# khuzema-h/marl-gym-pybullet-drones

Measured on NVIDIA B200. Metric: drone_substeps_per_sec, higher is better.
Workload: dtype f32

## Files before the change

include/batch_drones.h:

```cpp
#ifndef BATCH_DRONES_H_
#define BATCH_DRONES_H_

#include <stdint.h>

#ifdef __cplusplus
extern "C" {
#endif

#define BD_VERSION 1

enum { BD_TASK_HOVER = 0, BD_TASK_MULTIHOVER = 1, BD_TASK_SPIRAL = 2,
       BD_TASK_MEETUP = 3, BD_TASK_FLOCK = 4, BD_TASK_LEADERFOLLOWER = 5 };
enum { BD_ACT_RPM = 0, BD_ACT_ONE_D_RPM = 1, BD_ACT_PID = 2, BD_ACT_VEL = 3, BD_ACT_ONE_D_PID = 4 };
enum { BD_MODEL_CF2X = 0, BD_MODEL_CF2P = 1, BD_MODEL_RACE = 2 };
enum { BD_F32 = 0, BD_F64 = 1 };
enum { BD_AERO_GND = 1, BD_AERO_DRAG = 2, BD_AERO_DW = 4 };
enum { BD_INTEGRATOR_QUAT = 0, BD_INTEGRATOR_EULER = 1 };
enum { BD_RESET_FIXED = 0, BD_RESET_JITTER_PHILOX = 1, BD_RESET_JITTER_BUFFER = 2 };

enum {
  BD_OK = 0,
  BD_EINVAL = -1,
  BD_ECUDA = -2,
  BD_ENOMEM = -3
// ... 58 lines not shown
int bd_set_step_many_mode(bd_handle* h, int mode);
int bd_stream_gate(const uint32_t* flag_mapped, void* stream);

int bd_get_rng_state(const bd_handle* h, uint64_t* state4);
int bd_set_rng_state(bd_handle* h, const uint64_t* state4);

int bd_debug_set_tile_epoch(bd_handle* h, int tile, int value, void* stream);

int bd_get_state(bd_handle* h, void* state20_dev, void* rates_dev, int32_t* step_counter_dev,
                 void* stream);

int bd_set_state(bd_handle* h, const void* kin13_dev, const void* targets_dev,
                 const int32_t* step_counter_dev, void* stream);

int bd_get_targets(bd_handle* h, void* targets_dev, void* stream);

int bd_episode_stats(bd_handle* h, double* stats3_dev, int reset, void* stream);

int bd_get_controller_state(bd_handle* h, void* ctrl9_dev, void* stream);
int bd_set_controller_state(bd_handle* h, const void* ctrl9_dev, void* stream);

int bd_set_action_f32(bd_handle* h, int is_f32);

int bd_obs_dim(const bd_handle* h);
int bd_act_dim(const bd_handle* h);
int bd_action_buffer_size(const bd_handle* h);
int bd_substeps(const bd_handle* h);
int64_t bd_launch_count(const bd_handle* h);
const char* bd_last_error(void);
int bd_version(void);

typedef struct bd_actor bd_actor;
int bd_actor_create(int obs_dim, int hidden, int act_dim, int device, bd_actor** out);
void bd_actor_destroy(bd_actor* a);
int bd_actor_set_weights(bd_actor* a, const float* w1, const float* b1, const float* w2, const float* b2,
                         const float* w3, const float* b3, const float* logstd, void* stream);
int bd_actor_forward(bd_actor* a, const float* obs_dev, int64_t rows, const float* noise_dev, uint64_t seed,
                     uint64_t offset, float* act_dev, float* logp_dev, float* mean_dev, void* stream);
int bd_actor_set_trace(bd_actor* a, long long* trace_dev);
int bd_actor_set_input_norm(bd_actor* a, const float* mean_dev, const float* rstd_dev, int period, float clip);
int64_t bd_actor_launch_count(const bd_actor* a);
const char* bd_actor_last_error(void);

typedef struct bd_rms bd_rms;
int bd_rms_create(int cols, int device, double count0, double eps, bd_rms** out);
void bd_rms_destroy(bd_rms* r);
// ... 59 lines not shown
```

marl_gym_pybullet_drones_b200/_native.py:

```python
from __future__ import annotations

import ctypes as C
import os

_HERE = os.path.dirname(os.path.abspath(__file__))
LIB_PATH = os.path.join(_HERE, "libbatchdrones.so")

BD_TASK = {"hover": 0, "multihover": 1, "spiral": 2, "meetup": 3, "flock": 4, "leaderfollower": 5}
BD_ACT = {"rpm": 0, "one_d_rpm": 1, "pid": 2, "vel": 3, "one_d_pid": 4}
BD_MODEL = {"cf2x": 0, "cf2p": 1, "racer": 2}
BD_PRECISION = {"fp32": 0, "fp64": 1}
BD_INTEGRATOR = {"quat": 0, "euler": 1}
BD_RESET = {"fixed": 0, "jitter_philox": 1, "jitter_buffer": 2}

EXPORTS = (
    "bd_create", "bd_destroy", "bd_set_init_poses", "bd_set_jitter", "bd_reset", "bd_step",
    "bd_step_host", "bd_step_host_compact", "bd_step_many", "bd_set_step_many_mode", "bd_stream_gate", "bd_get_rng_state", "bd_set_rng_state",
    "bd_debug_set_tile_epoch", "bd_get_state", "bd_set_state", "bd_get_targets", "bd_episode_stats",
    "bd_get_controller_state", "bd_set_controller_state", "bd_set_action_f32", "bd_obs_dim", "bd_act_dim",
    "bd_action_buffer_size", "bd_substeps", "bd_launch_count", "bd_last_error", "bd_version",
    "bd_actor_create", "bd_actor_destroy", "bd_actor_set_weights", "bd_actor_forward", "bd_actor_set_trace", "bd_actor_launch_count",
    "bd_actor_last_error", "bd_actor_set_input_norm",
    "bd_rms_create", "bd_rms_destroy", "bd_rms_update", "bd_rms_batch_moments", "bd_rms_merge_moments", "bd_rms_normalize", "bd_rms_get", "bd_rms_set",
    "bd_rms_launch_count", "bd_rms_last_error",
    "bd_ppo_net_create", "bd_ppo_net_destroy", "bd_ppo_net_param_count", "bd_ppo_net_stats", "bd_ppo_net_pack", "bd_ppo_forward", "bd_ppo_sample", "bd_ppo_set_trace", "bd_ppo_set_train_mode", "bd_ppo_set_forward_mode",
    "bd_ppo_grad", "bd_ppo_adam_step", "bd_ppo_gae", "bd_ppo_adv_stats", "bd_ppo_launch_count", "bd_ppo_last_error",
    "bd_peer_create", "bd_peer_destroy", "bd_peer_handle_size", "bd_peer_get_handle", "bd_peer_open", "bd_peer_data", "bd_peer_allreduce",
    "bd_peer_unmap", "bd_peer_launch_count", "bd_peer_last_error",
)


class BdConfig(C.Structure):

    _fields_ = [
        ("struct_size", C.c_int32), ("device", C.c_int32),
        ("n_envs", C.c_int32), ("n_drones", C.c_int32),
        ("task", C.c_int32), ("act_type", C.c_int32), ("drone_model", C.c_int32),
        ("precision", C.c_int32), ("aero_flags", C.c_int32), ("integrator", C.c_int32),
        ("pyb_freq", C.c_int32), ("ctrl_freq", C.c_int32),
        ("auto_reset", C.c_int32), ("reset_mode", C.c_int32),
        ("action_is_f32", C.c_int32), ("keep_ang_vel", C.c_int32),
# ... 54 lines not shown
    lib.bd_get_rng_state.argtypes = [vp, C.POINTER(C.c_uint64)]
    lib.bd_get_rng_state.restype = C.c_int
    lib.bd_set_rng_state.argtypes = [vp, C.POINTER(C.c_uint64)]
    lib.bd_set_rng_state.restype = C.c_int
    lib.bd_debug_set_tile_epoch.argtypes = [vp, C.c_int, C.c_int, vp]
    lib.bd_debug_set_tile_epoch.restype = C.c_int
    lib.bd_get_state.argtypes = [vp, vp, vp, vp, vp]
    lib.bd_get_state.restype = C.c_int
    lib.bd_set_state.argtypes = [vp, vp, vp, vp, vp]
    lib.bd_set_state.restype = C.c_int
    lib.bd_get_targets.argtypes = [vp, vp, vp]
    lib.bd_get_targets.restype = C.c_int
    lib.bd_episode_stats.argtypes = [vp, vp, C.c_int, vp]
    lib.bd_episode_stats.restype = C.c_int
    lib.bd_get_controller_state.argtypes = [vp, vp, vp]
    lib.bd_get_controller_state.restype = C.c_int
    lib.bd_set_controller_state.argtypes = [vp, vp, vp]
    lib.bd_set_controller_state.restype = C.c_int
    lib.bd_set_action_f32.argtypes = [vp, C.c_int]
    lib.bd_set_action_f32.restype = C.c_int
    for name in ("bd_obs_dim", "bd_act_dim", "bd_action_buffer_size", "bd_substeps"):
        getattr(lib, name).argtypes = [vp]
        getattr(lib, name).restype = C.c_int
    lib.bd_launch_count.argtypes = [vp]
    lib.bd_launch_count.restype = C.c_int64
    lib.bd_last_error.argtypes = []
    lib.bd_last_error.restype = C.c_char_p
    lib.bd_version.argtypes = []
    lib.bd_version.restype = C.c_int
    lib.bd_actor_create.argtypes = [C.c_int, C.c_int, C.c_int, C.c_int, C.POINTER(vp)]
    lib.bd_actor_create.restype = C.c_int
    lib.bd_actor_destroy.argtypes = [vp]
    lib.bd_actor_destroy.restype = None
    lib.bd_actor_set_weights.argtypes = [vp] + [vp] * 7 + [vp]
    lib.bd_actor_set_weights.restype = C.c_int
    lib.bd_actor_forward.argtypes = [vp, vp, C.c_int64, vp, C.c_uint64, C.c_uint64, vp, vp, vp, vp]
    lib.bd_actor_forward.restype = C.c_int
    lib.bd_actor_set_trace.argtypes = [vp, vp]
    lib.bd_actor_set_trace.restype = C.c_int
    lib.bd_actor_launch_count.argtypes = [vp]
    lib.bd_actor_launch_count.restype = C.c_int64
    lib.bd_actor_last_error.argtypes = []
    lib.bd_actor_last_error.restype = C.c_char_p
    lib.bd_actor_set_input_norm.argtypes = [vp, vp, vp, C.c_int, C.c_float]
    lib.bd_actor_set_input_norm.restype = C.c_int
    lib.bd_rms_create.argtypes = [C.c_int, C.c_int, C.c_double, C.c_double, C.POINTER(vp)]
# ... 81 lines not shown
```

marl_gym_pybullet_drones_b200/csrc/bd_api.cu:

```cuda
#include <cuda_runtime.h>
#include <math.h>
#include <stdarg.h>
#include <stdio.h>
#include <stdlib.h>
#include <string.h>

#include <new>
#include <vector>

#include "../../include/batch_drones.h"
#include "bd_params.h"

namespace {

thread_local char g_err[512] = "";

int fail(int code, const char* fmt, ...) {
  va_list ap;
  va_start(ap, fmt);
  vsnprintf(g_err, sizeof(g_err), fmt, ap);
  va_end(ap);
  return code;
}

// ... 15 lines not shown
  }
  ~DeviceGuard() {
    if (prev >= 0 && prev != target) cudaSetDevice(prev);
  }
  int target = -1;
};

}

struct bd_handle {
  bd_config cfg;
  int S = 0, A = 0, B = 0, D = 0, E = 0;
  int EW = 1;
  long long n_total = 0;
  size_t real = 4;
  bd::LaunchSpec spec{};
  void *s0 = nullptr, *s1 = nullptr, *s2 = nullptr, *s3 = nullptr, *s4 = nullptr;
  float* hist = nullptr;
  int* stepc = nullptr;
  int* gsteps = nullptr;
  int* tile_epoch = nullptr;
  unsigned long long* finished = nullptr;
  int pipeline = 0;
  float* ep_ret = nullptr;
  double* ep_acc = nullptr;
  void* ctrl = nullptr;
  void* init_xyz = nullptr;
  void* init_rpy = nullptr;
  int init_env_stride = 0;
  void* jitter = nullptr;
  void* h_actions = nullptr;
  float* h_obs = nullptr;
  void* h_reward = nullptr;
  uint8_t *h_term = nullptr, *h_trunc = nullptr;
  float* h_tobs = nullptr;
  cudaStream_t hs_a = nullptr, hs_b = nullptr;
  cudaEvent_t hs_start = nullptr, hs_done = nullptr, hs_chunk[8] = {};
  int64_t launches = 0;
  long long total_steps = 0;
  bool graph_mode = false;
  int reset_epoch = 0;
  uint32_t philox_base = 0;
  int many_mode = 0;
  bool poisoned = false;
  int* c_blockcnt = nullptr;
  int* c_total = nullptr;
// ... 1 lines not shown
  float* c_rows_dev = nullptr;
  int c_cap_dev = 0;
  cudaEvent_t hs_compact = nullptr;
  int* c_host[2] = {nullptr, nullptr};
  float* c_rows_host[2] = {nullptr, nullptr};
  int c_cap[2] = {0, 0};
  int c_flip = 0;
  bd::Params<float> pf{};
  bd::Params<double> pd{};
};

namespace {

template <typename R>
void fill_params(const bd_handle* h, bd::Params<R>& P) {
  const bd_config& c = h->cfg;
  using R4 = typename bd::V4<R>::type;
  P.N = c.n_envs; P.M = c.n_drones; P.S = h->S; P.A = h->A; P.B = h->B; P.D = h->D;
  P.E = h->E; P.EW = h->EW; P.n_total = h->n_total;
  P.s0 = (R4*)h->s0; P.s1 = (R4*)h->s1; P.s2 = (R4*)h->s2; P.s3 = (R4*)h->s3; P.s4 = (R4*)h->s4;
  P.hist = h->hist; P.stepc = h->stepc; P.gsteps = h->gsteps; P.tile_epoch = h->tile_epoch; P.finished = h->finished;
  P.step_tiles = h->spec.impl == 1 ? (h->cfg.n_envs + 4 * h->EW - 1) / (4 * h->EW) : (h->cfg.n_envs + h->E - 1) / h->E;
  P.pipeline = h->pipeline; P.pipe_wait = 0; P.early_prefetch = 0; P.ep_ret = h->ep_ret; P.ep_acc = h->ep_acc;
  P.ctrl = (R*)h->ctrl;
  P.act_type = c.act_type; P.ctrl_reset = c.ctrl_reset_on_reset;
  P.ctrl_dt = (R)(1.0 / c.ctrl_freq);
  P.ctrl_gravity = (R)(c.g * c.ctrl_mass);
  P.ctrl_4kf = (R)(4 * c.ctrl_kf);
  P.speed_limit = (R)c.speed_limit; P.speed_limit_f = (float)c.speed_limit;
  P.init_xyz = (const R*)h->init_xyz; P.init_rpy = (const R*)h->init_rpy;
  P.init_env_stride = h->init_env_stride;
  P.jitter = (const R*)h->jitter;
  P.actions = nullptr; P.obs = nullptr; P.reward = nullptr; P.terminated = nullptr;
  P.truncated = nullptr; P.terminal_obs = nullptr; P.reset_mask = nullptr;
  const double gravity = c.g * c.mass;
  const double hover_rpm = sqrt(gravity / (4 * c.kf));
  const double max_rpm = sqrt((c.thrust2weight * gravity) / (4 * c.kf));
  const double max_thrust = 4 * c.kf * max_rpm * max_rpm;
  const double gnd_h_clip =
      0.25 * c.prop_radius * sqrt((15 * max_rpm * max_rpm * c.kf * c.gnd_eff_coeff) / max_thrust);
  P.dt = (R)(1.0 / c.pyb_freq);
  P.hover_rpm = (R)hover_rpm;
  P.kf = (R)c.kf; P.km = (R)c.km;
  P.arm = (R)(c.drone_model == BD_MODEL_CF2P ? c.arm : c.arm / sqrt(2.0));
  P.inv_m = (R)(1.0 / c.mass);
  P.gravity = (R)gravity;
// ... 183 lines not shown
  h->spec.device = cfg->device;
  const bool swarm = cfg->task >= BD_TASK_MEETUP;
  h->spec.generic = (cfg->aero_flags != 0 || cfg->integrator != BD_INTEGRATOR_QUAT || cfg->keep_ang_vel || pid_act || swarm) ? 1 : 0;
  {
    const int m = cfg->n_drones;
    const bool pow2 = (m & (m - 1)) == 0 && m <= 32;
    h->EW = m <= 32 ? 32 / m : 1;
    const char* force = getenv("BD_STEP_IMPL");
    const bool plain = cfg->integrator == BD_INTEGRATOR_QUAT && !cfg->keep_ang_vel;
    h->spec.impl = (cfg->precision == BD_F32 && plain && m <= 32 && (pow2 || !swarm) && !pid_act) ? 1 : 0;
    if (force && strcmp(force, "cta") == 0) h->spec.impl = 0;
    const char* pdl = getenv("BD_PDL");
    h->spec.pdl = (pdl && strcmp(pdl, "0") == 0) ? 0 : 1;
    const char* pl = getenv("BD_PIPELINE");
    h->pipeline = (h->spec.pdl && !(pl && strcmp(pl, "0") == 0)) ? 1 : 0;
  }

  const size_t smem = bd::step_smem_bytes(cfg->precision, h->A, h->B, h->D, cfg->task);
  cudaDeviceProp prop;
  cudaError_t pe = cudaGetDeviceProperties(&prop, cfg->device);
  if (pe != cudaSuccess) { delete h; return fail(BD_ECUDA, "cudaGetDeviceProperties: %s", cudaGetErrorString(pe)); }
  if (h->spec.impl == 1 && (size_t)(4 * h->EW) * cfg->n_drones * h->D * 4 > prop.sharedMemPerBlockOptin) h->spec.impl = 0;
  h->spec.sm_count = prop.multiProcessorCount;
  if (smem > prop.sharedMemPerBlockOptin) {
    delete h;
    return fail(BD_EINVAL, "bd_create: the history staging tile needs %zu B of shared memory (> %zu)", smem,
                (size_t)prop.sharedMemPerBlockOptin);
  }

  const size_t plane = (size_t)h->n_total * 4 * h->real;
  cudaError_t e = cudaSuccess;
  auto alloc = [&](void** p, size_t bytes) {
    if (e == cudaSuccess) e = cudaMalloc(p, bytes);
    if (e == cudaSuccess) e = cudaMemset(*p, 0, bytes);
  };
  alloc(&h->s0, plane); alloc(&h->s1, plane); alloc(&h->s2, plane); alloc(&h->s3, plane);
  if (cfg->keep_ang_vel) alloc(&h->s4, plane);
  alloc((void**)&h->hist, (size_t)h->B * h->n_total * h->A * sizeof(float));
  alloc((void**)&h->stepc, (size_t)cfg->n_envs * sizeof(int));
  alloc((void**)&h->gsteps, 16 * sizeof(int));
  alloc((void**)&h->tile_epoch, (size_t)epoch_tiles(h) * sizeof(int));
  alloc((void**)&h->finished, sizeof(unsigned long long));
  if (cfg->track_episodes) alloc((void**)&h->ep_ret, (size_t)cfg->n_envs * sizeof(float));
  alloc((void**)&h->ep_acc, 3 * sizeof(double));
  if (pid_act) alloc(&h->ctrl, (size_t)bd::kCtrlPlanesHost * h->n_total * h->real);
  if (e != cudaSuccess) {
// ... 476 lines not shown
  if (!h) return fail(BD_EINVAL, "bd_set_action_f32: null handle");
  if (h->cfg.precision == BD_F32 && !is_f32)
    return fail(BD_EINVAL, "bd_set_action_f32: BD_F32 handles take float actions only");
  h->cfg.action_is_f32 = is_f32 ? 1 : 0;
  if (h->h_actions) {
    DeviceGuard guard(h->cfg.device);
    cudaFree(h->h_actions); cudaFree(h->h_obs); cudaFree(h->h_reward); cudaFree(h->h_term); cudaFree(h->h_trunc);
    h->h_actions = nullptr; h->h_obs = nullptr; h->h_reward = nullptr; h->h_term = nullptr; h->h_trunc = nullptr;
  }
  refresh_params(h);
  return BD_OK;
}

int bd_episode_stats(bd_handle* h, double* stats3_dev, int reset, void* stream) {
  if (!h) return fail(BD_EINVAL, "bd_episode_stats: null handle");
  if (!h->ep_ret) return fail(BD_EINVAL, "bd_episode_stats: the handle was created with track_episodes = 0");
  DeviceGuard guard(h->cfg.device);
  cudaError_t e = bd::launch_episode_stats(h->ep_acc, stats3_dev, reset, (cudaStream_t)stream);
  h->launches++;
  if (e != cudaSuccess) return fail(BD_ECUDA, "episode_stats kernel launch failed: %s", cudaGetErrorString(e));
  return BD_OK;
}

int bd_obs_dim(const bd_handle* h) { return h ? h->D : BD_EINVAL; }
int bd_act_dim(const bd_handle* h) { return h ? h->A : BD_EINVAL; }
int bd_action_buffer_size(const bd_handle* h) { return h ? h->B : BD_EINVAL; }
int bd_substeps(const bd_handle* h) { return h ? h->S : BD_EINVAL; }
int64_t bd_launch_count(const bd_handle* h) { return h ? h->launches : 0; }

}
```

marl_gym_pybullet_drones_b200/csrc/bd_device.cuh:

```cuda
#pragma once
#include <cuda_runtime.h>
#include <math.h>
#include <stdint.h>

#include "bd_params.h"

namespace bd {

enum { TASK_HOVER = 0, TASK_MULTIHOVER = 1, TASK_SPIRAL = 2,
       TASK_SWARM = 3, TASK_MEETUP = 3, TASK_FLOCK = 4, TASK_LEADERFOLLOWER = 5 };
enum { MODEL_CF2X = 0, MODEL_CF2P = 1, MODEL_RACE = 2 };
enum { AERO_GND = 1, AERO_DRAG = 2, AERO_DW = 4 };
enum { RESET_FIXED = 0, RESET_PHILOX = 1, RESET_BUFFER = 2 };

__device__ __forceinline__ float  sqrt_(float x)  { return sqrtf(x); }
__device__ __forceinline__ double sqrt_(double x) { return sqrt(x); }
__device__ __forceinline__ float  exp_(float x)  { return expf(x); }
__device__ __forceinline__ double exp_(double x) { return exp(x); }
__device__ __forceinline__ float  atan2_(float y, float x)  { return atan2f(y, x); }
__device__ __forceinline__ double atan2_(double y, double x) { return atan2(y, x); }
__device__ __forceinline__ float  asin_(float x)  { return asinf(x); }
__device__ __forceinline__ double asin_(double x) { return asin(x); }
__device__ __forceinline__ void sincos_(float x, float* s, float* c)  { sincosf(x, s, c); }
__device__ __forceinline__ void sincos_(double x, double* s, double* c) { sincos(x, s, c); }
__device__ __forceinline__ float  abs_(float x)  { return fabsf(x); }
__device__ __forceinline__ double abs_(double x) { return fabs(x); }

__device__ __forceinline__ float4  make4(float a, float b, float c, float d)   { return make_float4(a, b, c, d); }
__device__ __forceinline__ double4 make4(double a, double b, double c, double d) { return make_double4(a, b, c, d); }

template <int BYTES>
__device__ __forceinline__ void cp_async(void* smem_dst, const void* gmem_src) {
  unsigned d = static_cast<unsigned>(__cvta_generic_to_shared(smem_dst));
  if constexpr (BYTES == 16) {
    asm volatile("cp.async.cg.shared.global [%0], [%1], 16;\n" ::"r"(d), "l"(gmem_src) : "memory");
  } else {
    asm volatile("cp.async.ca.shared.global [%0], [%1], %2;\n" ::"r"(d), "l"(gmem_src), "n"(BYTES) : "memory");
  }
}
__device__ __forceinline__ void cp_async_commit() { asm volatile("cp.async.commit_group;\n" ::: "memory"); }
__device__ __forceinline__ void cp_async_wait_all() { asm volatile("cp.async.wait_group 0;\n" ::: "memory"); }

__device__ __forceinline__ void philox4x32_10(uint32_t c[4], uint32_t k0, uint32_t k1) {
#pragma unroll
  for (int r = 0; r < 10; ++r) {
    const uint32_t hi0 = __umulhi(0xD2511F53u, c[0]), lo0 = 0xD2511F53u * c[0];
    const uint32_t hi1 = __umulhi(0xCD9E8D57u, c[2]), lo1 = 0xCD9E8D57u * c[2];
    const uint32_t n0 = hi1 ^ c[1] ^ k0, n2 = hi0 ^ c[3] ^ k1;
    c[0] = n0; c[1] = lo1; c[2] = n2; c[3] = lo0;
    k0 += 0x9E3779B9u; k1 += 0xBB67AE85u;
  }
}
__device__ __forceinline__ float  u01(uint32_t a, uint32_t, float)  { return (a >> 8) * (1.0f / 16777216.0f); }
__device__ __forceinline__ double u01(uint32_t a, uint32_t b, double) {
  return ((a >> 5) * 67108864.0 + (b >> 6)) * (1.0 / 9007199254740992.0);
}

template <typename R>
__device__ __forceinline__ void quat_to_mat(R x, R y, R z, R w, R m[9]) {
  const R d = x * x + y * y + z * z + w * w;
// ... 618 lines not shown
    R ir = clip_(c[3 + k] - re[k] * dt, R(-1500), R(1500));
    if (k < 2) ir = clip_(ir, R(-1), R(1));
    c[3 + k] = ir;
    const R itor = k == 2 ? R(500) : R(0);
    tq[k] = clip_((-(ptor[k] * re[k]) + dtor[k] * rate_e) + itor * ir, R(-3200), R(3200));
  }
  const R mix[4][3] = {{R(-.5), R(-.5), R(-1)}, {R(-.5), R(.5), R(1)}, {R(.5), R(.5), R(-1)}, {R(.5), R(-.5), R(1)}};
#pragma unroll
  for (int k = 0; k < 4; ++k) {
    const R pwm = clip_(thrust + ((mix[k][0] * tq[0] + mix[k][1] * tq[1]) + mix[k][2] * tq[2]), R(20000), R(65535));
    rpm[k] = R(0.2685) * pwm + R(4070.3);
  }
}

__device__ __forceinline__ void bulk_store_s2g(void* gdst, const void* ssrc, uint32_t bytes) {
  const unsigned s = static_cast<unsigned>(__cvta_generic_to_shared(ssrc));
  uint64_t policy;
  asm volatile("createpolicy.fractional.L2::evict_first.b64 %0, 1.0;\n" : "=l"(policy));
  asm volatile("cp.async.bulk.global.shared::cta.bulk_group.L2::cache_hint [%0], [%1], %2, %3;\n" ::"l"(gdst), "r"(s),
               "r"(bytes), "l"(policy)
               : "memory");
  asm volatile("cp.async.bulk.commit_group;\n" ::: "memory");
}
__device__ __forceinline__ void bulk_wait_read0() { asm volatile("cp.async.bulk.wait_group.read 0;\n" ::: "memory"); }
__device__ __forceinline__ void bulk_wait_all0() { asm volatile("cp.async.bulk.wait_group 0;\n" ::: "memory"); }
__device__ __forceinline__ void fence_proxy_async_smem() { asm volatile("fence.proxy.async.shared::cta;\n" ::: "memory"); }

template <int A, bool VEC>
__device__ __forceinline__ void history_run(float*& dst, const float* src, size_t plane, int n) {
#pragma unroll 2
  for (int j = 0; j < n; ++j) {
    if constexpr (VEC) cp_async<16>(dst, src);
    else {
#pragma unroll
      for (int k = 0; k < A; ++k) cp_async<4>(dst + k, src + k);
    }
    dst += A;
    src += plane;
  }
}

template <typename R, int A, bool VEC>
__device__ __forceinline__ void issue_history(const Params<R>& P, long long g, int head, float* myrow,
                                              int j0, int j1) {
  if (g < P.n_total) {
    const size_t plane = (size_t)P.n_total * A;
    const float* base = P.hist + (size_t)g * A;
    float* dst = myrow + 12 + j0 * A;
    const int s0 = head + 1 + j0;
    const int n = j1 - j0;
    if (s0 >= P.B) {
      history_run<A, VEC>(dst, base + (size_t)(s0 - P.B) * plane, plane, n);
    } else {
      const int n1 = min(n, P.B - s0);
      history_run<A, VEC>(dst, base + (size_t)s0 * plane, plane, n1);
      history_run<A, VEC>(dst, base, plane, n - n1);
    }
  }
}

__device__ __forceinline__ int ld_acquire_gpu(const int* p) {
  int v;
  asm volatile("ld.acquire.gpu.global.s32 %0, [%1];\n" : "=r"(v) : "l"(p) : "memory");
  return v;
}
__device__ __forceinline__ int ld_relaxed_gpu(const int* p) {
  int v;
  asm volatile("ld.relaxed.gpu.global.s32 %0, [%1];\n" : "=r"(v) : "l"(p) : "memory");
  return v;
}
__device__ __forceinline__ unsigned long long ld_relaxed_gpu_u64(const unsigned long long* p) {
  unsigned long long v;
  asm volatile("ld.relaxed.gpu.global.u64 %0, [%1];\n" : "=l"(v) : "l"(p) : "memory");
  return v;
}
__device__ __forceinline__ void st_release_gpu(int* p, int v) {
  asm volatile("st.release.gpu.global.s32 [%0], %1;\n" ::"l"(p), "r"(v) : "memory");
}

// ... 38 lines not shown
```

marl_gym_pybullet_drones_b200/csrc/bd_params.h:

```cpp
#pragma once
#include <cuda_runtime.h>
#include <stdint.h>

namespace bd {

constexpr int kBlock = 128;
constexpr int kMaxDrones = 128;
constexpr int kMaxJitterTries = 64;
constexpr int kCtrlPlanesHost = 13;

template <typename Real> struct V4;
template <> struct V4<float>  { using type = float4;  };
template <> struct V4<double> { using type = double4; };

template <typename Real>
struct Params {
  int N, M, S, A, B, D, E;
  int EW;
  long long n_total;
  typename V4<Real>::type *s0, *s1, *s2, *s3, *s4;
  float* hist;
  int* stepc;
  int* gsteps;
  float* ep_ret;
// ... 17 lines not shown
  Real sp_R, sp_omega, sp_vz, sp_cx, sp_cy;
  double pyb_freq, episode_len;
  int trunc_counter;
  int model, aero, integrator, auto_reset, reset_mode, action_is_f32, keep_angv;
  int task;
  int act_type, ctrl_reset;
  Real ctrl_dt, ctrl_gravity, ctrl_4kf, speed_limit;
  float speed_limit_f;
  int host_total;
  int host_head;
  int total_wrap;
  int* tile_epoch;
  unsigned long long* finished;
  long long step_tiles;
  int pipeline;
  int pipe_wait;
  int early_prefetch;
  int block0, grid_blocks;
  int advance;
  int reset_epoch;
  unsigned long long seed;
  int obs_aligned;
  uint32_t philox_base;
};

struct LaunchSpec {
  int task, act_a, precision, generic, device;
  int pdl;
  int impl;
  int sm_count;
};

cudaError_t launch_step_tile(int task, int act_a, const Params<float>& P, const LaunchSpec& ls, cudaStream_t st);
cudaError_t launch_step_tile_many(int task, int act_a, const Params<float>& P, int k, long long act_step, long long obs_step,
                                  long long out_step, const LaunchSpec& ls, cudaStream_t st);
cudaError_t launch_step(const LaunchSpec& ls, const void* params, cudaStream_t st);
cudaError_t launch_reset(const LaunchSpec& ls, const void* params, cudaStream_t st);
cudaError_t launch_get_state(int precision, const void* params, void* state20, void* rates,
                             int32_t* step_counter, cudaStream_t st);
cudaError_t launch_set_state(int precision, const void* params, const void* kin13,
                             const void* targets, const int32_t* step_counter, cudaStream_t st);
cudaError_t launch_get_targets(int precision, const void* params, void* targets, cudaStream_t st);
cudaError_t launch_ctrl_state(int precision, const void* params, void* dst, const void* src, int write,
                              cudaStream_t st);
cudaError_t launch_episode_stats(double* ep_acc, double* out3, int reset, cudaStream_t st);
size_t step_smem_bytes(int precision, int A, int B, int D, int task);
// ... 8 lines not shown
```

marl_gym_pybullet_drones_b200/csrc/bd_step_tile.cuh:

```cuda
#pragma once
#include "bd_device.cuh"

namespace bd {

template <int A>
struct TileIn {
  float4 s0, s1, s2, s3;
  float4 act;
  int stepc;
  float ep_ret;
};

template <int A>
__device__ __forceinline__ void load_state(const Params<float>& P, long long g, int env, bool active, TileIn<A>& in) {
  if (active) {
    in.s0 = P.s0[g]; in.s1 = P.s1[g]; in.s2 = P.s2[g]; in.s3 = P.s3[g];
    in.stepc = P.stepc[env];
    in.ep_ret = P.ep_ret != nullptr ? P.ep_ret[env] : 0.f;
  } else {
    in.s0 = in.s1 = in.s2 = in.s3 = make_float4(0.f, 0.f, 0.f, 0.f);
    in.s1.z = 1.0f;
    in.stepc = 0;
    in.ep_ret = 0.f;
  }
}
template <int A>
__device__ __forceinline__ void load_action(const Params<float>& P, long long g, bool active, TileIn<A>& in) {
  if (active) {
    if constexpr (A == 4) in.act = reinterpret_cast<const float4*>(P.actions)[g];
    else in.act = make_float4(reinterpret_cast<const float*>(P.actions)[g], 0.f, 0.f, 0.f);
  } else {
    in.act = make_float4(0.f, 0.f, 0.f, 0.f);
  }
}

__device__ __forceinline__ float swarm_reward_shfl(const Params<float>& P, const Drone<float>& d, float roll, float pitch,
                                                   int lane, int M, int drone, int& flags) {
  const unsigned full = 0xffffffffu;
  const int base = lane & ~(M - 1);
  const bool tilt = fabsf(roll) > .4f || fabsf(pitch) > .4f;
  flags = 0;
  float contrib = 0.f;
  if (P.task == TASK_MEETUP) {
    const int src = base | (M - 1 - drone);
    const float ox = __shfl_sync(full, d.px, src), oy = __shfl_sync(full, d.py, src), oz = __shfl_sync(full, d.pz, src);
    if (drone < M / 2) {
      const float dx = d.px - ox, dy = d.py - oy, dz = d.pz - oz;
      const float dist = sqrtf(dx * dx + dy * dy + dz * dz);
      contrib = (-1.f * (dist * dist)) * 2.f;
      if (dist > 0.1f) flags |= 4;
    }
    if (fabsf(d.px) > 5.0f || fabsf(d.py) > 5.0f || d.pz > 3.0f || d.pz < 0.1f || tilt) flags |= 2;
  } else if (P.task == TASK_LEADERFOLLOWER) {
// ... 53 lines not shown
}

template <int TASK, int A, bool VEC, int AERO>
__global__ void __launch_bounds__(kBlock, 6)
step_kernel_tile(const __grid_constant__ Params<float> P) {
  extern __shared__ __align__(128) unsigned char smem_raw[];
  const int tid = threadIdx.x, lane = tid & 31;
  const int M = P.M, B = P.B, D = P.D, EW = P.EW;
  const bool pow2 = (M & (M - 1)) == 0;
  constexpr bool vec = VEC;
  float* tile_s = reinterpret_cast<float*>(smem_raw);
  const int env_w = pow2 ? (lane >> (31 - __clz(M))) : lane / M;
  const int group_base = env_w * M;
  const int drone = lane - group_base;
  const int tile = blockIdx.x + P.block0;
  const int env_l = (tid >> 5) * EW + env_w;
  const int env = tile * (4 * EW) + env_l;
  const bool active = env_w < EW && env < P.N;
  const long long g0 = (long long)tile * (4 * EW) * M;
  const long long g = (long long)env * M + drone;
  float* myrow = tile_s + (size_t)(env_w < EW ? env_l * M + drone : 0) * D;
  const bool jit = (TASK == TASK_MULTIHOVER) && (P.reset_mode != RESET_FIXED);
  const long long gh = active ? g : P.n_total;

  pdl_launch_dependents();
  int total, head;
  const bool pipe = P.pipe_wait && P.host_total >= 0;
  if (pipe) {
    total = P.host_total;
    head = P.host_head;
    if (pipe_gate(P, tile, total, tid)) pdl_wait();
    issue_history<float, A, VEC>(P, gh, head, myrow, 0, B - 2);
  } else if (P.host_total >= 0 && P.early_prefetch) {
    total = P.host_total;
    head = P.host_head;
    issue_history<float, A, VEC>(P, gh, head, myrow, 0, B - 2);
    pdl_wait();
  } else {
    pdl_wait();
    total = P.host_total >= 0 ? P.host_total : P.gsteps[0];
    head = total % B;
    issue_history<float, A, VEC>(P, gh, head, myrow, 0, B - 2);
  }
  TileIn<A> cur;
  load_state<A>(P, g, env, active, cur);
  issue_history<float, A, VEC>(P, gh, head, myrow, B - 2, B - 1);
  cp_async_commit();
  load_action<A>(P, g, active, cur);
  const int stepc = cur.stepc;
  float last_sum = 0.f;
  if constexpr (AERO == 2) {
    if ((P.aero & AERO_DRAG) && active && stepc > 0) {
      const int prev = head == 0 ? B - 1 : head - 1;
      const float* lp = P.hist + ((size_t)prev * P.n_total + g) * A;
      if constexpr (A == 4) {
        const float4 pa = *reinterpret_cast<const float4*>(lp);
        last_sum = (__fadd_rn(1.0f, __fmul_rn(0.05f, pa.x)) + __fadd_rn(1.0f, __fmul_rn(0.05f, pa.y))) +
                   (__fadd_rn(1.0f, __fmul_rn(0.05f, pa.z)) + __fadd_rn(1.0f, __fmul_rn(0.05f, pa.w)));
      } else {
        last_sum = 4.0f * __fadd_rn(1.0f, __fmul_rn(0.05f, lp[0]));
      }
    }
  }

  Drone<float> d;
  d.px = cur.s0.x; d.py = cur.s0.y; d.pz = cur.s0.z; d.qx = cur.s0.w;
  d.qy = cur.s1.x; d.qz = cur.s1.y; d.qw = cur.s1.z; d.vx = cur.s1.w;
  d.vy = cur.s2.x; d.vz = cur.s2.y; d.wx = cur.s2.z; d.wy = cur.s2.w;
  d.wz = cur.s3.x; d.tx = cur.s3.y; d.ty = cur.s3.z; d.tz = cur.s3.w;
  float onep[4];
  if constexpr (A == 4) {
// ... 8 lines not shown
  float avx = 0.f, avy = 0.f, avz = 0.f;
  fast_substeps<AERO>(P, d, onep, avx, avy, avz, group_base, drone, last_sum);
  float roll, pitch, yaw;
  quat_to_euler_fast(d.qx, d.qy, d.qz, d.qw, roll, pitch, yaw);

  cp_async_wait_all();
  float contrib = 0.f;
  int flags = 0;
  if (active) {
    if (vec) {
      float4* r4 = reinterpret_cast<float4*>(myrow);
      r4[0] = make_float4(d.px, d.py, d.pz, roll);
      r4[1] = make_float4(pitch, yaw, d.vx, d.vy);
      r4[2] = make_float4(d.vz, avx, avy, avz);
    } else {
      myrow[0] = d.px; myrow[1] = d.py; myrow[2] = d.pz; myrow[3] = roll; myrow[4] = pitch; myrow[5] = yaw;
      myrow[6] = d.vx; myrow[7] = d.vy; myrow[8] = d.vz; myrow[9] = avx; myrow[10] = avy; myrow[11] = avz;
    }
    if constexpr (TASK != TASK_SWARM)
      task_terms<float, TASK>(P, d, roll, pitch, stepc, drone, myrow + 12 + B * A, contrib, flags);
    if constexpr (A == 4) {
      if (vec) *reinterpret_cast<float4*>(myrow + 12 + (B - 1) * 4) = cur.act;
      else { float* o = myrow + 12 + (B - 1) * 4; o[0] = cur.act.x; o[1] = cur.act.y; o[2] = cur.act.z; o[3] = cur.act.w; }
      *reinterpret_cast<float4*>(P.hist + ((size_t)head * P.n_total + g) * 4) = cur.act;
    } else {
      myrow[12 + B - 1] = cur.act.x;
      P.hist[(size_t)head * P.n_total + g] = cur.act.x;
    }
  }

  float swarm_reward_env = 0.f;
  if constexpr (TASK == TASK_SWARM) {
    int fl = 0;
    swarm_reward_env = swarm_reward_shfl(P, d, roll, pitch, lane, M, drone, fl);
    flags = active ? fl : 0;
  }
  if (pow2) {
#pragma unroll 1
    for (int o = M >> 1; o > 0; o >>= 1) {
      contrib += __shfl_xor_sync(0xffffffffu, contrib, o);
      flags |= __shfl_xor_sync(0xffffffffu, flags, o);
    }
  } else {
    const float c0 = contrib;
    const int f0 = flags;
#pragma unroll 1
    for (int o = 1; o < M; ++o) {
      int t = drone + o;
      t -= (t >= M) ? M : 0;
      contrib += __shfl_sync(0xffffffffu, c0, group_base + t);
      flags |= __shfl_sync(0xffffffffu, f0, group_base + t);
    }
  }
  const float reward = (TASK == TASK_SWARM) ? swarm_reward_env : ((TASK == TASK_HOVER) ? contrib : contrib / (float)M);
  const bool time_up = stepc >= P.trunc_counter;
  const bool terminated = (TASK == TASK_SWARM) ? (P.task == TASK_MEETUP && (flags & 4) == 0) : (flags & 1) != 0;
  const bool truncated = ((flags & 2) != 0) || time_up;
  const bool done_reset = active && (terminated || truncated) && P.auto_reset;
  if (active && drone == 0) {
    P.reward[env] = reward;
    P.terminated[env] = terminated ? 1 : 0;
    P.truncated[env] = truncated ? 1 : 0;
    P.stepc[env] = done_reset ? 0 : stepc + P.S;
    if (P.ep_ret != nullptr) {
      float ep = cur.ep_ret + reward;
      if (terminated || truncated) {
        atomicAdd(P.ep_acc + 0, (double)ep);
        atomicAdd(P.ep_acc + 1, (double)(stepc / P.S + 1));
        atomicAdd(P.ep_acc + 2, 1.0);
        ep = 0.f;
      }
      P.ep_ret[env] = ep;
    }
  }

  if (__any_sync(0xffffffffu, done_reset)) {
    float cx = 0.f, cy = 0.f, cz = 0.f;
    if (jit) {
      const long long ib = (long long)env * P.init_env_stride + drone * 3;
      bool retry = done_reset;
#pragma unroll 1
      for (int attempt = 0; attempt <= kMaxJitterTries; ++attempt) {
        const bool last = attempt == kMaxJitterTries;
        if (retry) {
          float j0 = 0.f, j1 = 0.f, j2 = 0.f;
          if (!last) {
            if (P.reset_mode == RESET_BUFFER && P.jitter != nullptr) {
              j0 = P.jitter[g * 3]; j1 = P.jitter[g * 3 + 1]; j2 = P.jitter[g * 3 + 2];
            } else {
              uint32_t c[4] = {(uint32_t)env, (uint32_t)total + P.philox_base, (uint32_t)(attempt * M + drone), 0u};
              uint32_t c2[4] = {c[0], c[1], c[2], 1u};
              philox4x32_10(c, (uint32_t)P.seed, (uint32_t)(P.seed >> 32));
              philox4x32_10(c2, (uint32_t)P.seed, (uint32_t)(P.seed >> 32));
              j0 = -0.25f + 0.5f * u01(c[0], c[1], 0.f);
              j1 = -0.25f + 0.5f * u01(c[2], c[3], 0.f);
// ... 42 lines not shown
      for (int k = 0; k < 12; ++k) myrow[k] = kin[k];
      if (TASK == TASK_SPIRAL) {
        float rp[3], rv[3], sphi, cphi;
        spiral_reference(P, 0, drone, rp, rv, sphi, cphi);
        spiral_extras(myrow + 12 + B * A, d, rp, rv, sphi, cphi);
      }
    }
  }

  const long long left = P.n_total - g0;
  const int tile_rows = 4 * EW * M;
  const int rows = (int)(left < (long long)tile_rows ? left : (long long)tile_rows);
  const uint32_t bytes = (uint32_t)rows * (uint32_t)D * 4u;
  float* gobs = P.obs + (size_t)g0 * D;
  const bool bulk = P.obs_aligned && (bytes & 15u) == 0;
  if (bulk) fence_proxy_async_smem();
  __syncthreads();
  if (bulk) {
    if (tid == 0) bulk_store_s2g(gobs, tile_s, bytes);
  } else {
    for (int i = tid; i < rows * D; i += kBlock) gobs[i] = tile_s[i];
  }
  if (active) {
    P.s0[g] = make_float4(d.px, d.py, d.pz, d.qx);
    P.s1[g] = make_float4(d.qy, d.qz, d.qw, d.vx);
    P.s2[g] = make_float4(d.vy, d.vz, d.wx, d.wy);
    P.s3[g] = make_float4(d.wz, d.tx, d.ty, d.tz);
  }
  if (P.pipeline) {
    __syncthreads();
    if (tid == 0) {
      if (bulk) bulk_wait_all0();
      if (P.host_total >= 0) {
        if (tile == 0) P.gsteps[0] = (total + 1 >= P.total_wrap) ? 0 : total + 1;
      } else {
        const unsigned ticket = atomicAdd(reinterpret_cast<unsigned*>(P.gsteps + 1), 1u);
        if (ticket == gridDim.x - 1) {
          P.gsteps[1] = 0;
          if (P.advance) P.gsteps[0] = (total + 1 >= P.total_wrap) ? 0 : total + 1;
        }
      }
      st_release_gpu(P.tile_epoch + tile, total + 1);
      atomicAdd(P.finished, 1ull);
    }
    return;
  }
  if (tid == 0) {
    const unsigned ticket = atomicAdd(reinterpret_cast<unsigned*>(P.gsteps + 1), 1u);
    if (ticket == gridDim.x - 1) {
      P.gsteps[1] = 0;
// ... 287 lines not shown
```

Measured before the change: 61.04 billion.

## Add L2 cache eviction-priority hints for state, action history and actions

Adds a host-side planner that sizes how much persistent drone state and how many action-history slots fit in about 30% of L2, and per-access createpolicy cache hints in the step-tile kernel. State loads and stores and recent history slots get evict_last, older slots and the one-time action reads get evict_first, so data reused on the next step stays resident in L2 instead of being refetched from HBM. The hinted loads use inline PTX with volatile asm and memory clobbers, which may limit compiler scheduling. The policy can be overridden through the BD_L2_KEEP environment variable.

Measured after the change: 64.81 billion, median of 6. +6.2%, better.

```diff
diff --git a/include/batch_drones.h b/include/batch_drones.h
--- a/include/batch_drones.h
+++ b/include/batch_drones.h
@@ -104,6 +104,10 @@
 
 int bd_set_action_f32(bd_handle* h, int is_f32);
 
+int bd_l2_plan(int n_envs, int n_drones, int act_dim, int buf_slots, int track_episodes, int64_t l2_bytes,
+               const char* force, int* keep_state, int* keep_slots);
+int bd_l2_policy(const bd_handle* h, int* keep_state, int* keep_slots);
+
 int bd_obs_dim(const bd_handle* h);
 int bd_act_dim(const bd_handle* h);
 int bd_action_buffer_size(const bd_handle* h);
diff --git a/marl_gym_pybullet_drones_b200/_native.py b/marl_gym_pybullet_drones_b200/_native.py
--- a/marl_gym_pybullet_drones_b200/_native.py
+++ b/marl_gym_pybullet_drones_b200/_native.py
@@ -16,7 +16,7 @@
 EXPORTS = (
     "bd_create", "bd_destroy", "bd_set_init_poses", "bd_set_jitter", "bd_reset", "bd_step",
     "bd_step_host", "bd_step_host_compact", "bd_step_many", "bd_set_step_many_mode", "bd_stream_gate", "bd_get_rng_state", "bd_set_rng_state",
-    "bd_debug_set_tile_epoch", "bd_get_state", "bd_set_state", "bd_get_targets", "bd_episode_stats",
+    "bd_debug_set_tile_epoch", "bd_l2_plan", "bd_l2_policy", "bd_get_state", "bd_set_state", "bd_get_targets", "bd_episode_stats",
     "bd_get_controller_state", "bd_set_controller_state", "bd_set_action_f32", "bd_obs_dim", "bd_act_dim",
     "bd_action_buffer_size", "bd_substeps", "bd_launch_count", "bd_last_error", "bd_version",
     "bd_actor_create", "bd_actor_destroy", "bd_actor_set_weights", "bd_actor_forward", "bd_actor_set_trace", "bd_actor_launch_count",
@@ -117,6 +117,11 @@
     for name in ("bd_obs_dim", "bd_act_dim", "bd_action_buffer_size", "bd_substeps"):
         getattr(lib, name).argtypes = [vp]
         getattr(lib, name).restype = C.c_int
+    ip = C.POINTER(C.c_int)
+    lib.bd_l2_plan.argtypes = [C.c_int, C.c_int, C.c_int, C.c_int, C.c_int, C.c_int64, C.c_char_p, ip, ip]
+    lib.bd_l2_plan.restype = C.c_int
+    lib.bd_l2_policy.argtypes = [vp, ip, ip]
+    lib.bd_l2_policy.restype = C.c_int
     lib.bd_launch_count.argtypes = [vp]
     lib.bd_launch_count.restype = C.c_int64
     lib.bd_last_error.argtypes = []
diff --git a/marl_gym_pybullet_drones_b200/csrc/bd_api.cu b/marl_gym_pybullet_drones_b200/csrc/bd_api.cu
--- a/marl_gym_pybullet_drones_b200/csrc/bd_api.cu
+++ b/marl_gym_pybullet_drones_b200/csrc/bd_api.cu
@@ -61,6 +61,7 @@
   int* tile_epoch = nullptr;
   unsigned long long* finished = nullptr;
   int pipeline = 0;
+  int l2_keep_state = 0, l2_keep_slots = 0;
   float* ep_ret = nullptr;
   double* ep_acc = nullptr;
   void* ctrl = nullptr;
@@ -108,6 +109,7 @@
   P.hist = h->hist; P.stepc = h->stepc; P.gsteps = h->gsteps; P.tile_epoch = h->tile_epoch; P.finished = h->finished;
   P.step_tiles = h->spec.impl == 1 ? (h->cfg.n_envs + 4 * h->EW - 1) / (4 * h->EW) : (h->cfg.n_envs + h->E - 1) / h->E;
   P.pipeline = h->pipeline; P.pipe_wait = 0; P.early_prefetch = 0; P.ep_ret = h->ep_ret; P.ep_acc = h->ep_acc;
+  P.l2_keep_state = h->l2_keep_state; P.l2_keep_slots = h->l2_keep_slots;
   P.ctrl = (R*)h->ctrl;
   P.act_type = c.act_type; P.ctrl_reset = c.ctrl_reset_on_reset;
   P.ctrl_dt = (R)(1.0 / c.ctrl_freq);
@@ -337,6 +339,11 @@
   if (pe != cudaSuccess) { delete h; return fail(BD_ECUDA, "cudaGetDeviceProperties: %s", cudaGetErrorString(pe)); }
   if (h->spec.impl == 1 && (size_t)(4 * h->EW) * cfg->n_drones * h->D * 4 > prop.sharedMemPerBlockOptin) h->spec.impl = 0;
   h->spec.sm_count = prop.multiProcessorCount;
+  if (h->spec.impl == 1) {
+    const int rc = bd_l2_plan(cfg->n_envs, cfg->n_drones, h->A, h->B, cfg->track_episodes, prop.l2CacheSize,
+                              getenv("BD_L2_KEEP"), &h->l2_keep_state, &h->l2_keep_slots);
+    if (rc) { delete h; return rc; }
+  }
   if (smem > prop.sharedMemPerBlockOptin) {
     delete h;
     return fail(BD_EINVAL, "bd_create: the history staging tile needs %zu B of shared memory (> %zu)", smem,
@@ -859,6 +866,44 @@
   return BD_OK;
 }
 
+int bd_l2_plan(int n_envs, int n_drones, int act_dim, int buf_slots, int track_episodes, int64_t l2_bytes,
+               const char* force, int* keep_state, int* keep_slots) {
+  if (!keep_state || !keep_slots) return fail(BD_EINVAL, "bd_l2_plan: null output");
+  if (n_envs < 1 || n_drones < 1 || act_dim < 1 || buf_slots < 1 || l2_bytes < 0)
+    return fail(BD_EINVAL, "bd_l2_plan: bad shape");
+  *keep_state = 0;
+  *keep_slots = 0;
+  if (force && *force) {
+    if (strcmp(force, "off") == 0) return BD_OK;
+    *keep_state = 1;
+    if (strcmp(force, "state") == 0) return BD_OK;
+    char* end = nullptr;
+    const long k = strtol(force, &end, 10);
+    if (end == force || *end != '\0' || k < 0) {
+      *keep_state = 0;
+      return fail(BD_EINVAL, "BD_L2_KEEP=%s: expected off, state or a slot count", force);
+    }
+    *keep_slots = (int)(k < buf_slots - 1 ? k : buf_slots - 1);
+    return BD_OK;
+  }
+  const long long n = (long long)n_envs * n_drones;
+  const long long state = n * 64 + (long long)n_envs * (track_episodes ? 8 : 4);
+  const long long slot = n * act_dim * 4;
+  const long long budget = l2_bytes * 3 / 10;
+  if (state > budget) return BD_OK;
+  *keep_state = 1;
+  const long long k = (budget - state) / slot;
+  *keep_slots = (int)(k < buf_slots - 1 ? k : buf_slots - 1);
+  return BD_OK;
+}
+
+int bd_l2_policy(const bd_handle* h, int* keep_state, int* keep_slots) {
+  if (!h || !keep_state || !keep_slots) return fail(BD_EINVAL, "bd_l2_policy: null argument");
+  *keep_state = h->l2_keep_state;
+  *keep_slots = h->l2_keep_slots;
+  return BD_OK;
+}
+
 int bd_obs_dim(const bd_handle* h) { return h ? h->D : BD_EINVAL; }
 int bd_act_dim(const bd_handle* h) { return h ? h->A : BD_EINVAL; }
 int bd_action_buffer_size(const bd_handle* h) { return h ? h->B : BD_EINVAL; }
diff --git a/marl_gym_pybullet_drones_b200/csrc/bd_device.cuh b/marl_gym_pybullet_drones_b200/csrc/bd_device.cuh
--- a/marl_gym_pybullet_drones_b200/csrc/bd_device.cuh
+++ b/marl_gym_pybullet_drones_b200/csrc/bd_device.cuh
@@ -36,6 +36,16 @@
     asm volatile("cp.async.cg.shared.global [%0], [%1], 16;\n" ::"r"(d), "l"(gmem_src) : "memory");
   } else {
     asm volatile("cp.async.ca.shared.global [%0], [%1], %2;\n" ::"r"(d), "l"(gmem_src), "n"(BYTES) : "memory");
+  }
+}
+template <int BYTES>
+__device__ __forceinline__ void cp_async_hint(void* smem_dst, const void* gmem_src, uint64_t pol) {
+  unsigned d = static_cast<unsigned>(__cvta_generic_to_shared(smem_dst));
+  if constexpr (BYTES == 16) {
+    asm volatile("cp.async.cg.shared.global.L2::cache_hint [%0], [%1], 16, %2;\n" ::"r"(d), "l"(gmem_src), "l"(pol) : "memory");
+  } else {
+    asm volatile("cp.async.ca.shared.global.L2::cache_hint [%0], [%1], %2, %3;\n" ::"r"(d), "l"(gmem_src), "n"(BYTES), "l"(pol)
+                 : "memory");
   }
 }
 __device__ __forceinline__ void cp_async_commit() { asm volatile("cp.async.commit_group;\n" ::: "memory"); }
@@ -700,39 +710,108 @@
                : "memory");
   asm volatile("cp.async.bulk.commit_group;\n" ::: "memory");
 }
+__device__ __forceinline__ uint64_t l2_pol_last() {
+  uint64_t p;
+  asm("createpolicy.fractional.L2::evict_last.b64 %0, 1.0;\n" : "=l"(p));
+  return p;
+}
+__device__ __forceinline__ uint64_t l2_pol_first() {
+  uint64_t p;
+  asm("createpolicy.fractional.L2::evict_first.b64 %0, 1.0;\n" : "=l"(p));
+  return p;
+}
+__device__ __forceinline__ uint64_t l2_pol_normal() {
+  uint64_t p;
+  asm("createpolicy.fractional.L2::evict_normal.b64 %0, 1.0;\n" : "=l"(p));
+  return p;
+}
+struct L2Hints {
+  uint64_t state;
+  uint64_t slot_keep;
+  uint64_t slot_drop;
+  uint64_t once;
+  int keep_slots;
+};
+template <typename R>
+__device__ __forceinline__ L2Hints l2_hints(const Params<R>& P) {
+  const uint64_t last = l2_pol_last(), first = l2_pol_first(), normal = l2_pol_normal();
+  const bool on = P.l2_keep_state || P.l2_keep_slots > 0;
+  return {P.l2_keep_state ? last : normal, last, on ? first : normal, first, P.l2_keep_slots};
+}
+__device__ __forceinline__ uint64_t l2_slot_pol(const L2Hints& h, int age) { return age < h.keep_slots ? h.slot_keep : h.slot_drop; }
+
+__device__ __forceinline__ float4 ld_hint(const float4* p, uint64_t pol) {
+  float4 v;
+  asm volatile("ld.global.L2::cache_hint.v4.f32 {%0, %1, %2, %3}, [%4], %5;\n"
+               : "=f"(v.x), "=f"(v.y), "=f"(v.z), "=f"(v.w) : "l"(p), "l"(pol) : "memory");
+  return v;
+}
+__device__ __forceinline__ float ld_hint(const float* p, uint64_t pol) {
+  float v;
+  asm volatile("ld.global.L2::cache_hint.f32 %0, [%1], %2;\n" : "=f"(v) : "l"(p), "l"(pol) : "memory");
+  return v;
+}
+__device__ __forceinline__ int ld_hint(const int* p, uint64_t pol) {
+  int v;
+  asm volatile("ld.global.L2::cache_hint.s32 %0, [%1], %2;\n" : "=r"(v) : "l"(p), "l"(pol) : "memory");
+  return v;
+}
+__device__ __forceinline__ void st_hint(float4* p, float4 v, uint64_t pol) {
+  asm volatile("st.global.L2::cache_hint.v4.f32 [%0], {%1, %2, %3, %4}, %5;\n" ::"l"(p), "f"(v.x), "f"(v.y), "f"(v.z), "f"(v.w),
+               "l"(pol)
+               : "memory");
+}
+__device__ __forceinline__ void st_hint(float* p, float v, uint64_t pol) {
+  asm volatile("st.global.L2::cache_hint.f32 [%0], %1, %2;\n" ::"l"(p), "f"(v), "l"(pol) : "memory");
+}
+__device__ __forceinline__ void st_hint(int* p, int v, uint64_t pol) {
+  asm volatile("st.global.L2::cache_hint.s32 [%0], %1, %2;\n" ::"l"(p), "r"(v), "l"(pol) : "memory");
+}
+
 __device__ __forceinline__ void bulk_wait_read0() { asm volatile("cp.async.bulk.wait_group.read 0;\n" ::: "memory"); }
 __device__ __forceinline__ void bulk_wait_all0() { asm volatile("cp.async.bulk.wait_group 0;\n" ::: "memory"); }
 __device__ __forceinline__ void fence_proxy_async_smem() { asm volatile("fence.proxy.async.shared::cta;\n" ::: "memory"); }
 
-template <int A, bool VEC>
-__device__ __forceinline__ void history_run(float*& dst, const float* src, size_t plane, int n) {
+template <int A, bool VEC, bool HINT>
+__device__ __forceinline__ void history_run(float*& dst, const float* src, size_t plane, int n, int& age, const L2Hints& h) {
 #pragma unroll 2
   for (int j = 0; j < n; ++j) {
-    if constexpr (VEC) cp_async<16>(dst, src);
-    else {
+    if constexpr (HINT) {
+      const uint64_t pol = l2_slot_pol(h, age);
+      if constexpr (VEC) cp_async_hint<16>(dst, src, pol);
+      else {
 #pragma unroll
-      for (int k = 0; k < A; ++k) cp_async<4>(dst + k, src + k);
+        for (int k = 0; k < A; ++k) cp_async_hint<4>(dst + k, src + k, pol);
+      }
+    } else {
+      if constexpr (VEC) cp_async<16>(dst, src);
+      else {
+#pragma unroll
+        for (int k = 0; k < A; ++k) cp_async<4>(dst + k, src + k);
+      }
     }
     dst += A;
     src += plane;
-  }
-}
-
-template <typename R, int A, bool VEC>
+    --age;
+  }
+}
+
+template <typename R, int A, bool VEC, bool HINT = false>
 __device__ __forceinline__ void issue_history(const Params<R>& P, long long g, int head, float* myrow,
-                                              int j0, int j1) {
+                                              int j0, int j1, const L2Hints& h = L2Hints{}) {
   if (g < P.n_total) {
     const size_t plane = (size_t)P.n_total * A;
     const float* base = P.hist + (size_t)g * A;
     float* dst = myrow + 12 + j0 * A;
     const int s0 = head + 1 + j0;
     const int n = j1 - j0;
+    int age = P.B - 1 - j0;
     if (s0 >= P.B) {
-      history_run<A, VEC>(dst, base + (size_t)(s0 - P.B) * plane, plane, n);
+      history_run<A, VEC, HINT>(dst, base + (size_t)(s0 - P.B) * plane, plane, n, age, h);
     } else {
       const int n1 = min(n, P.B - s0);
-      history_run<A, VEC>(dst, base + (size_t)s0 * plane, plane, n1);
-      history_run<A, VEC>(dst, base, plane, n - n1);
+      history_run<A, VEC, HINT>(dst, base + (size_t)s0 * plane, plane, n1, age, h);
+      history_run<A, VEC, HINT>(dst, base, plane, n - n1, age, h);
     }
   }
 }
diff --git a/marl_gym_pybullet_drones_b200/csrc/bd_params.h b/marl_gym_pybullet_drones_b200/csrc/bd_params.h
--- a/marl_gym_pybullet_drones_b200/csrc/bd_params.h
+++ b/marl_gym_pybullet_drones_b200/csrc/bd_params.h
@@ -63,6 +63,8 @@
   unsigned long long seed;
   int obs_aligned;
   uint32_t philox_base;
+  int l2_keep_state;
+  int l2_keep_slots;
 };
 
 struct LaunchSpec {
diff --git a/marl_gym_pybullet_drones_b200/csrc/bd_step_tile.cuh b/marl_gym_pybullet_drones_b200/csrc/bd_step_tile.cuh
--- a/marl_gym_pybullet_drones_b200/csrc/bd_step_tile.cuh
+++ b/marl_gym_pybullet_drones_b200/csrc/bd_step_tile.cuh
@@ -11,12 +11,20 @@
   float ep_ret;
 };
 
-template <int A>
-__device__ __forceinline__ void load_state(const Params<float>& P, long long g, int env, bool active, TileIn<A>& in) {
+template <int A, bool HINT = false>
+__device__ __forceinline__ void load_state(const Params<float>& P, long long g, int env, bool active, TileIn<A>& in,
+                                           const L2Hints& h = L2Hints{}) {
   if (active) {
-    in.s0 = P.s0[g]; in.s1 = P.s1[g]; in.s2 = P.s2[g]; in.s3 = P.s3[g];
-    in.stepc = P.stepc[env];
-    in.ep_ret = P.ep_ret != nullptr ? P.ep_ret[env] : 0.f;
+    if constexpr (HINT) {
+      in.s0 = ld_hint(P.s0 + g, h.state); in.s1 = ld_hint(P.s1 + g, h.state);
+      in.s2 = ld_hint(P.s2 + g, h.state); in.s3 = ld_hint(P.s3 + g, h.state);
+      in.stepc = ld_hint(P.stepc + env, h.state);
+      in.ep_ret = P.ep_ret != nullptr ? ld_hint(P.ep_ret + env, h.state) : 0.f;
+    } else {
+      in.s0 = P.s0[g]; in.s1 = P.s1[g]; in.s2 = P.s2[g]; in.s3 = P.s3[g];
+      in.stepc = P.stepc[env];
+      in.ep_ret = P.ep_ret != nullptr ? P.ep_ret[env] : 0.f;
+    }
   } else {
     in.s0 = in.s1 = in.s2 = in.s3 = make_float4(0.f, 0.f, 0.f, 0.f);
     in.s1.z = 1.0f;
@@ -24,11 +32,17 @@
     in.ep_ret = 0.f;
   }
 }
-template <int A>
-__device__ __forceinline__ void load_action(const Params<float>& P, long long g, bool active, TileIn<A>& in) {
+template <int A, bool HINT = false>
+__device__ __forceinline__ void load_action(const Params<float>& P, long long g, bool active, TileIn<A>& in,
+                                            const L2Hints& h = L2Hints{}) {
   if (active) {
-    if constexpr (A == 4) in.act = reinterpret_cast<const float4*>(P.actions)[g];
-    else in.act = make_float4(reinterpret_cast<const float*>(P.actions)[g], 0.f, 0.f, 0.f);
+    if constexpr (HINT) {
+      if constexpr (A == 4) in.act = ld_hint(reinterpret_cast<const float4*>(P.actions) + g, h.once);
+      else in.act = make_float4(ld_hint(reinterpret_cast<const float*>(P.actions) + g, h.once), 0.f, 0.f, 0.f);
+    } else {
+      if constexpr (A == 4) in.act = reinterpret_cast<const float4*>(P.actions)[g];
+      else in.act = make_float4(reinterpret_cast<const float*>(P.actions)[g], 0.f, 0.f, 0.f);
+    }
   } else {
     in.act = make_float4(0.f, 0.f, 0.f, 0.f);
   }
@@ -128,6 +142,7 @@
   float* myrow = tile_s + (size_t)(env_w < EW ? env_l * M + drone : 0) * D;
   const bool jit = (TASK == TASK_MULTIHOVER) && (P.reset_mode != RESET_FIXED);
   const long long gh = active ? g : P.n_total;
+  const L2Hints l2 = l2_hints(P);
 
   pdl_launch_dependents();
   int total, head;
@@ -136,23 +151,23 @@
     total = P.host_total;
     head = P.host_head;
     if (pipe_gate(P, tile, total, tid)) pdl_wait();
-    issue_history<float, A, VEC>(P, gh, head, myrow, 0, B - 2);
+    issue_history<float, A, VEC, true>(P, gh, head, myrow, 0, B - 2, l2);
   } else if (P.host_total >= 0 && P.early_prefetch) {
     total = P.host_total;
     head = P.host_head;
-    issue_history<float, A, VEC>(P, gh, head, myrow, 0, B - 2);
+    issue_history<float, A, VEC, true>(P, gh, head, myrow, 0, B - 2, l2);
     pdl_wait();
   } else {
     pdl_wait();
     total = P.host_total >= 0 ? P.host_total : P.gsteps[0];
     head = total % B;
-    issue_history<float, A, VEC>(P, gh, head, myrow, 0, B - 2);
+    issue_history<float, A, VEC, true>(P, gh, head, myrow, 0, B - 2, l2);
   }
   TileIn<A> cur;
-  load_state<A>(P, g, env, active, cur);
-  issue_history<float, A, VEC>(P, gh, head, myrow, B - 2, B - 1);
+  load_state<A, true>(P, g, env, active, cur, l2);
+  issue_history<float, A, VEC, true>(P, gh, head, myrow, B - 2, B - 1, l2);
   cp_async_commit();
-  load_action<A>(P, g, active, cur);
+  load_action<A, true>(P, g, active, cur, l2);
   const int stepc = cur.stepc;
   float last_sum = 0.f;
   if constexpr (AERO == 2) {
@@ -207,10 +222,10 @@
     if constexpr (A == 4) {
       if (vec) *reinterpret_cast<float4*>(myrow + 12 + (B - 1) * 4) = cur.act;
       else { float* o = myrow + 12 + (B - 1) * 4; o[0] = cur.act.x; o[1] = cur.act.y; o[2] = cur.act.z; o[3] = cur.act.w; }
-      *reinterpret_cast<float4*>(P.hist + ((size_t)head * P.n_total + g) * 4) = cur.act;
+      st_hint(reinterpret_cast<float4*>(P.hist + ((size_t)head * P.n_total + g) * 4), cur.act, l2_slot_pol(l2, 0));
     } else {
       myrow[12 + B - 1] = cur.act.x;
-      P.hist[(size_t)head * P.n_total + g] = cur.act.x;
+      st_hint(P.hist + (size_t)head * P.n_total + g, cur.act.x, l2_slot_pol(l2, 0));
     }
   }
 
@@ -246,7 +261,7 @@
     P.reward[env] = reward;
     P.terminated[env] = terminated ? 1 : 0;
     P.truncated[env] = truncated ? 1 : 0;
-    P.stepc[env] = done_reset ? 0 : stepc + P.S;
+    st_hint(P.stepc + env, done_reset ? 0 : stepc + P.S, l2.state);
     if (P.ep_ret != nullptr) {
       float ep = cur.ep_ret + reward;
       if (terminated || truncated) {
@@ -255,7 +270,7 @@
         atomicAdd(P.ep_acc + 2, 1.0);
         ep = 0.f;
       }
-      P.ep_ret[env] = ep;
+      st_hint(P.ep_ret + env, ep, l2.state);
     }
   }
 
@@ -344,10 +359,10 @@
     for (int i = tid; i < rows * D; i += kBlock) gobs[i] = tile_s[i];
   }
   if (active) {
-    P.s0[g] = make_float4(d.px, d.py, d.pz, d.qx);
-    P.s1[g] = make_float4(d.qy, d.qz, d.qw, d.vx);
-    P.s2[g] = make_float4(d.vy, d.vz, d.wx, d.wy);
-    P.s3[g] = make_float4(d.wz, d.tx, d.ty, d.tz);
+    st_hint(P.s0 + g, make_float4(d.px, d.py, d.pz, d.qx), l2.state);
+    st_hint(P.s1 + g, make_float4(d.qy, d.qz, d.qw, d.vx), l2.state);
+    st_hint(P.s2 + g, make_float4(d.vy, d.vz, d.wx, d.wy), l2.state);
+    st_hint(P.s3 + g, make_float4(d.wz, d.tx, d.ty, d.tz), l2.state);
   }
   if (P.pipeline) {
     __syncthreads();
```
